# Benjamin-Lee/circkit

Measured on NVIDIA B200. Metric: canonicalize+uniq records/sec, higher is better.
Workload: dtype u8

## Files before the change

### circkit_b200/csrc/ck_kernels.cuh

```cuda
#pragma once
#include "ck_hash.cuh"

namespace ck {

enum : int {
    CLS_W2S = 0,
    CLS_W2M = 1,
    CLS_C2A = 2,
    CLS_C2B = 3,
    CLS_W4 = 4,
    CLS_C4 = 5,
    CLS_W8 = 6,
    CLS_C8 = 7,
    CLS_HUGE = 8,
    CLS_EMPTY = 9,
    CLS_W2L = 10,
    CLS_W2X = 11,
    CLS_COUNT = 12
};
__host__ __device__ constexpr u32 cls_max_n(int c)
{
    return c == CLS_W2S ? 512u : c == CLS_W2M ? 2048u : c == CLS_W2L ? 4096u : c == CLS_W2X ? 8192u : c == CLS_C2A ? 65536u
         : c == CLS_C2B ? 425984u : c == CLS_W4 ? 2048u : c == CLS_C4 ? 212992u : c == CLS_W8 ? 1024u : c == CLS_C8 ? 106496u
         : c == CLS_EMPTY ? 0u : 0xffffffffu;
// ... 316 lines not shown
                    const u32 v = min(16u, rawlen - p);
                    u32 unit = prep_pack16(prep_load16(src16 + (p >> 4), sh, p + 16 < span));
                    if (v < 16) unit &= ~(0xffffffffu >> (2 * v));
                    dst32[p >> 4] = unit;
                }
            }
            continue;
        }
        if (cnt == rawlen && spanA <= 512) {
            const u32 p = 16 * lane;
            if (p < spanA) {
                const u32 lo = p < A ? A - p : 0u, hi = min(16u, spanA - p);
                if (hi - lo == 16) *reinterpret_cast<uint4 *>(gbase + p) = m1;
                else {
                    const u32 valid = (hi >= 16 ? 0xffffu : ((1u << hi) - 1u)) & ~((1u << lo) - 1u);
                    const u32 w[4] = {m1.x, m1.y, m1.z, m1.w};
                    u8 *g = gbase + p;
                    u32 vb = valid;
#pragma unroll
                    for (int i = 0; i < 4; i++)
                        if (((valid >> (4 * i)) & 15u) == 15u) { *reinterpret_cast<u32 *>(g + 4 * i) = w[i]; vb &= ~(15u << (4 * i)); }
                    prep_store_bytes(g, w, vb);
                }
            }
            continue;
        }
        u32 S = pack2 ? 0u : A;
        u32 done = 0;
        for (u32 base = 0; base < rawlen; base += 512) {
            const u32 p = base + 16 * lane;
            uint4 m = make_uint4(0, 0, 0, 0);
            u32 mask = 0;
            if (p < rawlen) {
                u32 f;
                prep_lookup(tab, prep_load16(src16 + (p >> 4), sh, p + 16 < span), 0u, min(16u, rawlen - p), m, f, mask);
            }
            const u32 kc = __popc(mask);
            u32 incl = kc;
#pragma unroll
            for (int d = 1; d < 32; d <<= 1) { const u32 t = __shfl_up_sync(CK_FULL, incl, d); if (lane >= (u32)d) incl += t; }
            const u32 T = __shfl_sync(CK_FULL, incl, 31);
            u32 idx = S + incl - kc;
            __syncwarp();
#pragma unroll
            for (int k = 0; k < 16; k++)
                if ((mask >> k) & 1u) stage[idx++] = (u8)prep_byte(m, k);
            __syncwarp();
            const u32 fill = S + T;
            if (pack2) {
                const u32 U = fill >> 4;
                for (u32 j = lane; j < U; j += 32) dst32[done + j] = prep_pack16(*reinterpret_cast<const uint4 *>(stage + 16 * j));
                const u32 r = fill & 15u;
                u8 c = 0;
                if (lane < r) c = stage[16 * U + lane];
                __syncwarp();
                if (lane < r) stage[lane] = c;
                done += U; S = r;
            } else {
                u8 *g = dstb + done - S;
                for (u32 w = lane; 16 * w < fill; w += 32) {
                    const u32 lo = max(16 * w, S), hi = min(16 * w + 16, fill);
                    if (hi - lo == 16) *reinterpret_cast<uint4 *>(g + 16 * w) = *reinterpret_cast<const uint4 *>(stage + 16 * w);
                    else for (u32 i = lo; i < hi; i++) g[i] = stage[i];
                }
                done += T; S = (u32)((size_t)(dstb + done) & 15u);
            }
        }
        __syncwarp();
        if (pack2 && S && lane == 0)
            dst32[done] = prep_pack16(*reinterpret_cast<const uint4 *>(stage)) & ~(0xffffffffu >> (2 * S));
        __syncwarp();
    }
}

struct ClassifyArgs {
    const u64 *offsets; const u32 *lens; const u8 *lane;
    u32 n_records;
    u32 *keys, *vals;
    u32 *counts;
    u32 direct_mask;
    u32 window_shift;
    u32 top_bit;
};
__global__ void __launch_bounds__(256) k_classify(ClassifyArgs a)
{
    __shared__ u32 cnt[16];
    if (threadIdx.x < 16) cnt[threadIdx.x] = 0;
    __syncthreads();
    const u32 nthreads = gridDim.x * blockDim.x;
    const u32 rounds = (a.n_records + nthreads - 1) / nthreads;
    for (u32 r = 0; r < rounds; r++) {
        const u32 i = r * nthreads + blockIdx.x * blockDim.x + threadIdx.x;
        int cls = -1;
        u32 n = 0;
        if (i < a.n_records) {
            n = a.lens ? a.lens[i] : (u32)(a.offsets[i + 1] - a.offsets[i]);
            const u32 bits = a.lane ? a.lane[i] : 2u;
            if (n == 0) cls = CLS_EMPTY;
            else if (bits == 2) cls = n <= cls_max_n(CLS_W2S) ? CLS_W2S : n <= cls_max_n(CLS_W2M) ? CLS_W2M
                                    : n <= cls_max_n(CLS_W2L) ? CLS_W2L : n <= cls_max_n(CLS_W2X) ? CLS_W2X
                                    : n <= cls_max_n(CLS_C2A) ? CLS_C2A : n <= cls_max_n(CLS_C2B) ? CLS_C2B : CLS_HUGE;
            else if (bits == 4 || bits == 3) cls = n <= cls_max_n(CLS_W4) ? CLS_W4 : n <= cls_max_n(CLS_C4) ? CLS_C4 : CLS_HUGE;
            else cls = n <= cls_max_n(CLS_W8) ? CLS_W8 : n <= cls_max_n(CLS_C8) ? CLS_C8 : CLS_HUGE;
        }
        if (a.direct_mask) {
            const u32 m = __ballot_sync(CK_FULL, cls >= 0 && !((a.direct_mask >> cls) & 1u));
            if (m && lane_id() == (u32)(__ffs(m) - 1)) atomicAdd(cnt + CLS_HUGE, __popc(m));
            continue;
        }
        if (cls >= 0) {
            const u32 msb = 31u - __clz(n | 1u);
            const u32 bin = (msb << 5) | ((((n << (31u - msb)) >> 29) & 3u) << 3);
            u32 key = (cls_rank(cls) << 10) | bin;
            if (a.window_shift < 32u) {
                const bool lane_cls = cls == CLS_W2S || cls == CLS_W2M || cls == CLS_W2L || cls == CLS_W2X;
                const u32 q = (msb << 2) | (((n << (31u - msb)) >> 29) & 3u);
                key = lane_cls ? (((i >> a.window_shift) << 5) | (q > 28u ? q - 28u : 0u)) : (key | (1u << a.top_bit));
            }
            a.keys[i] = key; a.vals[i] = i;
        }
        u32 todo = __ballot_sync(CK_FULL, cls >= 0);
        while (todo) {
            const int c = __shfl_sync(CK_FULL, cls, __ffs(todo) - 1);
            const u32 m = __ballot_sync(CK_FULL, cls == c);
            if (lane_id() == (u32)(__ffs(m) - 1)) atomicAdd(cnt + c, __popc(m));
            todo &= ~m;
        }
    }
    __syncthreads();
    if (threadIdx.x < 16 && cnt[threadIdx.x]) atomicAdd(a.counts + threadIdx.x, cnt[threadIdx.x]);
}
__global__ void k_list_starts(u32 *counts)
{
    if (threadIdx.x == 0) {
        u32 s = 0;
        for (u32 r = 0; r < (u32)CLS_COUNT; r++) {
            const int c = cls_of_rank(r);
            counts[16 + c] = s; counts[48 + c] = s;
            s += counts[c];
        }
        counts[12] = counts[CLS_W2S] + counts[CLS_W2M] + counts[CLS_W2L] + counts[CLS_W2X];
        counts[28] = counts[16 + CLS_W2S];
        counts[13] = counts[CLS_C2A] + counts[CLS_C2B];
        counts[29] = counts[16 + CLS_C2A];
    }
}

__device__ __forceinline__ u32 p2_last_unit(u32 n) { return max((2u * n + 143u) >> 4, (n >> 4) + 5u); }
__device__ __forceinline__ void extend_one(u64 *packed2, const u64 *offsets, const u32 *lens, u32 i, const u64 *dense, u32 dbl, u32 lane)
{
    const u64 off = offsets[i];
    const u32 n = lens ? lens[i] : (u32)(offsets[i + 1] - off);
    if (n == 0) return;
    u32 *U = reinterpret_cast<u32 *>(packed2 + p2_word(off, i, dbl));
    const u32 *S = dense ? reinterpret_cast<const u32 *>(dense + (off >> 5) + i) : U;
    const u32 jn = n >> 4, last = dbl ? p2_last_unit(n) : jn + 4;
    if (n >= 80) {
        for (u32 j = (dense ? 0u : jn) + lane; j <= last; j += 32) {
            const u32 r = (16u * j) % n;
            const u32 q = r >> 4, sh = 2u * (r & 15u);
            u32 w = __funnelshift_l(__ldcg(S + q + 1), __ldcg(S + q), sh);
            if (r + 16u > n) {
                const u32 k = n - r;
                w = (w & ~(0xffffffffu >> (2u * k))) | (__ldcg(S) >> (2u * k));
            }
            U[j] = w;
        }
    } else {
        for (u32 j = (dense ? 0u : jn) + lane; j <= last; j += 32) {
            u32 v = 0;
            for (u32 b = 0; b < 16; b++) {
                const u32 t = (16 * j + b) % n;
                v = (v << 2) | ((__ldcg(S + (t >> 4)) >> (30 - 2 * (t & 15))) & 3u);
            }
            __syncwarp(__activemask());
            U[j] = v;
        }
    }
    __syncwarp();
}
__global__ void __launch_bounds__(256) k_extend_packed2(u64 *packed2, const u64 *offsets, const u32 *lens, const u8 *lane_bits, u32 n_records,
                                                        const u64 *dense, u32 dbl)
{
    const u32 lane = lane_id();
    const u32 gw = (blockIdx.x * blockDim.x + threadIdx.x) >> 5, nw = (gridDim.x * blockDim.x) >> 5;
    if (n_records < 65536u) {
        for (u32 i = gw; i < n_records; i += nw) {
            if (lane_bits && lane_bits[i] != 2) continue;
            extend_one(packed2, offsets, lens, i, dense, dbl, lane);
        }
        return;
    }
    for (u32 i0 = 32u * gw; i0 < n_records; i0 += 32u * nw) {
        const u32 ii = i0 + lane;
        u32 m = __ballot_sync(CK_FULL, ii < n_records && (!lane_bits || lane_bits[ii] == 2));
        while (m) {
            const u32 i = i0 + (u32)__ffs(m) - 1u;
            m &= m - 1u;
            extend_one(packed2, offsets, lens, i, dense, dbl, lane);
        }
    }
}

__global__ void __launch_bounds__(256) k_scatter_lane_bytes(const u8 *lane_bytes, const u64 *lane_offsets, const u64 *offsets, const u32 *lens,
                                                            const u8 *lane_bits, u32 n_records, u8 *bytes)
{
    const u32 lane = lane_id();
    const u32 gw = (blockIdx.x * blockDim.x + threadIdx.x) >> 5, nw = (gridDim.x * blockDim.x) >> 5;
    for (u32 i = gw; i < n_records; i += nw) {
        if (lane_bits[i] == 2) continue;
        const u8 *src = lane_bytes + lane_offsets[i];
        u8 *dst = bytes + offsets[i];
        const u32 n = lens[i];
        for (u32 k = lane; k < n; k += 32) dst[k] = src[k];
    }
}

struct TableArgs {
    TableSlot *slots; u64 nslots;
    u64 *side_first;
    const u64 *hash; const u64 *index;
    u32 stride;
    u64 base_index; u32 n;
    u64 *slot_of;
    u64 *first_out;
    u32 *overflow;
    u64 *keys;
// ... 317 lines not shown
```

### circkit_b200/csrc/ck_lib.cu

```cuda
#include <algorithm>
#include <cstdio>
#include <cstdlib>
#include <cstring>
#include <mutex>
#include <new>
#include <string>
#include <vector>

#include <cub/device/device_radix_sort.cuh>
#include <cub/device/device_scan.cuh>
#include <cub/device/device_select.cuh>
#include <cub/iterator/counting_input_iterator.cuh>

#include "../../include/circkit_b200.h"
#include "ck_kernels.cuh"
#include "ck_warp2.cuh"
#include "ck_lane2.cuh"
#include "ck_stream2.cuh"
#include "ck_stream3.cuh"
#include "ck_seg2.cuh"
#include "ck_lane4.cuh"
#include "ck_synth.cuh"
#include "ck_monomerize.cuh"
#include "ck_fasta.cuh"
// ... 52 lines not shown
struct ExecScratch {
    u32 *tie[CLS_COUNT] = {};
    u64 *seg = nullptr;
    u32 *huge_x = nullptr, *huge_tie = nullptr;
    u64 huge_x_words = 0, huge_tie_words = 0;
    cudaStream_t side_stream[CLS_COUNT] = {};
    cudaEvent_t ev_fork = nullptr, ev_join[CLS_COUNT] = {};
};

struct Slot {
    cudaStream_t stream = nullptr;
    cudaEvent_t inserted = nullptr;
    u8 *d_raw = nullptr; u64 *d_off = nullptr; u64 *d_p2 = nullptr; u8 *d_norm = nullptr; u8 *d_p4 = nullptr;
    u32 *d_len = nullptr; u8 *d_lane = nullptr; u8 *d_out = nullptr; u32 *d_start = nullptr;
    u8 *d_strand = nullptr; u64 *d_hash = nullptr; u64 *d_first = nullptr; u64 *d_slotof = nullptr;
    u32 *d_lists = nullptr; u32 *d_counts = nullptr;
    u64 *d_dense = nullptr; u64 *d_laneoff = nullptr;
    u32 *h_counts = nullptr;
    ExecScratch scr;
    bool busy = false, uniq = false, mono = false;
    bool text = false;
    u32 cmd = 0;
    u8 *d_text = nullptr, *d_frame = nullptr;
    u64 *d_rstart = nullptr, *d_head = nullptr, *d_seq = nullptr, *d_len64 = nullptr, *d_fofs = nullptr, *d_meta = nullptr;
    u32 *d_tiles = nullptr;
    u32 dbl = 1;
    u64 longest = 0;
    u32 *sel = nullptr; u64 *coff = nullptr;
    u32 n = 0, flags = 0; u64 total = 0;
    u64 rec_mark = 0;
    bool defl = false;
    struct Deflate {
        cudaStream_t stream = nullptr;
        u64 cap = 0;
        u8 *buf = nullptr;
        u32 *kA = nullptr, *kB = nullptr, *vA = nullptr, *vB = nullptr;
        u32 *prev8 = nullptr, *prev4 = nullptr;
        u32 *seg = nullptr;
        u32 *out = nullptr, *result = nullptr;
        u32 *h_result = nullptr;
        void *tmp = nullptr; size_t tmp_bytes = 0;
        u64 n = 0;
    } z;
};

struct PeerGroup {
    u32 world = 1, rank = 0, cap = 0;
    u8 *block = nullptr; u64 block_bytes = 0, recv_bytes = 0, ret_bytes = 0;
    void *mapped[32] = {};
    bool exported = false, attached = false;
    u64 epoch[4] = {};
    u32 *pos[2] = {}; u32 *cursors[2] = {}; u64 *slot_of[2] = {};
    u64 *recv(u32 r, u32 slot) const { return reinterpret_cast<u64 *>((u8 *)mapped[r] + CK_PEER_HEADER_BYTES + (u64)slot * recv_bytes); }
    u64 *ret(u32 r, u32 slot) const { return reinterpret_cast<u64 *>((u8 *)mapped[r] + CK_PEER_HEADER_BYTES + 2 * recv_bytes + (u64)slot * ret_bytes); }
    u64 *counts(u32 r, u32 slot) const { return reinterpret_cast<u64 *>(mapped[r]) + CK_PEER_FLAG_WORDS + 32u * slot; }
};

}

struct ck_ctx {
    int device = 0;
    int num_sms = 148;
    ck_config cfg{};
    std::string err;
    Slot slot[2];
    ExecScratch dev_scr;
    cudaEvent_t last_insert = nullptr;
    bool have_last_insert = false;
    TableSlot *table = nullptr; u64 table_slots = 0; u64 *side = nullptr; u32 *d_overflow = nullptr;
    u64 *d_keys = nullptr;
    u64 grow_max = 0, grows = 0;
    u64 known_keys = 0, known_rec = 0, submitted_rec = 0;
    PeerGroup peer;
    std::mutex lib_mu;
    cudaStream_t lib_stream = nullptr;
    u8 *lib_h = nullptr, *lib_d = nullptr; size_t lib_h_bytes = 0, lib_d_bytes = 0;
    ExecScratch lib_scr;
    u64 launches = 0;
    bool attrs_set = false;
    u32 s3_debug = 0;
    bool l4_kernel = true;
    bool seg_kernel = true;
    int lane_kernel = 3;
    bool timing = false;
    std::vector<cudaEvent_t> ev_pairs[CLS_COUNT + 7];
};

namespace {

int fail(ck_ctx *ctx, int code, const char *what, cudaError_t e = cudaSuccess)
{
    std::string m = what;
    if (e != cudaSuccess) { m += ": "; m += cudaGetErrorString(e); }
    if (ctx) ctx->err = m; else g_init_error = m;
    return code;
}
#define CK_CUDA(ctx, call)                                                     \
    do {                                                                       \
        cudaError_t e__ = (call);                                              \
        if (e__ != cudaSuccess) return fail((ctx), CK_ERR_CUDA, #call, e__);   \
    } while (0)

void fill_tables(Tables &t, u8 secret[200])
{
    for (int c = 0; c < 256; c++) t.norm[c] = 'N';
    for (const char *p = "ACGTN-"; *p; p++) t.norm[(u8)*p] = (u8)*p;
    t.norm['a'] = 'A'; t.norm['c'] = 'C'; t.norm['g'] = 'G';
    t.norm['t'] = 'T'; t.norm['u'] = 'T'; t.norm['U'] = 'T';
    t.norm['.'] = '-'; t.norm['~'] = '-';
    t.norm[' '] = 0; t.norm['\t'] = 0; t.norm['\r'] = 0; t.norm['\n'] = 0;
    for (int c = 0; c < 256; c++) t.comp[c] = (u8)c;
    const char *a = "AGCTYRWSKMDVHBN", *b = "TCGARYWSMKHBDVN";
    for (int i = 0; a[i]; i++) { t.comp[(u8)a[i]] = (u8)b[i]; t.comp[(u8)a[i] + 32] = (u8)(b[i] + 32); }
    const char *alpha = "-ABCDGHKMNRSTVWY";
    for (int c = 0; c < 256; c++) t.code4[c] = 0xff;
    for (int i = 0; i < 16; i++) { t.sym4[i] = (u8)alpha[i]; t.code4[(u8)alpha[i]] = (u8)i; }
    for (int i = 0; i < 16; i++) t.comp4[i] = t.code4[t.comp[t.sym4[i]]];
    static const u8 sec[192] = {
        0xb8, 0xfe, 0x6c, 0x39, 0x23, 0xa4, 0x4b, 0xbe, 0x7c, 0x01, 0x81, 0x2c, 0xf7, 0x21, 0xad, 0x1c,
        0xde, 0xd4, 0x6d, 0xe9, 0x83, 0x90, 0x97, 0xdb, 0x72, 0x40, 0xa4, 0xa4, 0xb7, 0xb3, 0x67, 0x1f,
        0xcb, 0x79, 0xe6, 0x4e, 0xcc, 0xc0, 0xe5, 0x78, 0x82, 0x5a, 0xd0, 0x7d, 0xcc, 0xff, 0x72, 0x21,
        0xb8, 0x08, 0x46, 0x74, 0xf7, 0x43, 0x24, 0x8e, 0xe0, 0x35, 0x90, 0xe6, 0x81, 0x3a, 0x26, 0x4c,
        0x3c, 0x28, 0x52, 0xbb, 0x91, 0xc3, 0x00, 0xcb, 0x88, 0xd0, 0x65, 0x8b, 0x1b, 0x53, 0x2e, 0xa3,
        0x71, 0x64, 0x48, 0x97, 0xa2, 0x0d, 0xf9, 0x4e, 0x38, 0x19, 0xef, 0x46, 0xa9, 0xde, 0xac, 0xd8,
        0xa8, 0xfa, 0x76, 0x3f, 0xe3, 0x9c, 0x34, 0x3f, 0xf9, 0xdc, 0xbb, 0xc7, 0xc7, 0x0b, 0x4f, 0x1d,
        0x8a, 0x51, 0xe0, 0x4b, 0xcd, 0xb4, 0x59, 0x31, 0xc8, 0x9f, 0x7e, 0xc9, 0xd9, 0x78, 0x73, 0x64,
        0xea, 0xc5, 0xac, 0x83, 0x34, 0xd3, 0xeb, 0xc3, 0xc5, 0x81, 0xa0, 0xff, 0xfa, 0x13, 0x63, 0xeb,
        0x17, 0x0d, 0xdd, 0x51, 0xb7, 0xf0, 0xda, 0x49, 0xd3, 0x16, 0x55, 0x26, 0x29, 0xd4, 0x68, 0x9e,
        0x2b, 0x16, 0xbe, 0x58, 0x7d, 0x47, 0xa1, 0xfc, 0x8f, 0xf8, 0xb8, 0xd1, 0x7a, 0xd0, 0x31, 0xce,
        0x45, 0xcb, 0x3a, 0x8f, 0x95, 0x16, 0x04, 0x28, 0xaf, 0xd7, 0xfb, 0xca, 0xbb, 0x4b, 0x40, 0x7e,
    };
    memset(secret, 0, 200);
    memcpy(secret, sec, 192);
}

int alloc_scratch(ck_ctx *ctx, ExecScratch &s)
{
    CK_CUDA(ctx, cudaEventCreateWithFlags(&s.ev_fork, cudaEventDisableTiming));
    for (int c = 0; c < CLS_COUNT; c++) {
        CK_CUDA(ctx, cudaStreamCreateWithFlags(&s.side_stream[c], cudaStreamNonBlocking));
        CK_CUDA(ctx, cudaEventCreateWithFlags(&s.ev_join[c], cudaEventDisableTiming));
    }
    CK_CUDA(ctx, cudaMalloc(&s.seg, (size_t)2 * ctx->num_sms * CK_SEG_WARPS * CK_SEG_SCRATCH_U64 * 8));
    for (int c = 0; c < CLS_COUNT; c++) {
        if (kCls[c].bits == 0) continue;
        const u64 groups = (u64)kCls[c].ctas_per_sm * ctx->num_sms * (kCls[c].cta ? 1u : kCls[c].threads / 32u);
        CK_CUDA(ctx, cudaMalloc(&s.tie[c], groups * cls_tie_words(c) * 4));
    }
    return CK_OK;
}
void free_scratch(ExecScratch &s)
{
    for (int c = 0; c < CLS_COUNT; c++) {
        if (s.tie[c]) cudaFree(s.tie[c]);
        if (s.side_stream[c]) cudaStreamDestroy(s.side_stream[c]);
        if (s.ev_join[c]) cudaEventDestroy(s.ev_join[c]);
        s.tie[c] = nullptr; s.side_stream[c] = nullptr; s.ev_join[c] = nullptr;
    }
    if (s.ev_fork) cudaEventDestroy(s.ev_fork);
    if (s.seg) cudaFree(s.seg);
    if (s.huge_x) cudaFree(s.huge_x);
    if (s.huge_tie) cudaFree(s.huge_tie);
    s.huge_x = s.huge_tie = nullptr; s.huge_x_words = s.huge_tie_words = 0;
    s.ev_fork = nullptr; s.seg = nullptr;
}

template <typename K> int set_smem(ck_ctx *ctx, K kernel, u32 bytes)
{
    if (bytes > 48 * 1024) CK_CUDA(ctx, cudaFuncSetAttribute(kernel, cudaFuncAttributeMaxDynamicSharedMemorySize, (int)bytes));
    return CK_OK;
}
void s2_launch(ck_ctx *ctx, cudaStream_t st, const CanonArgs &a, int v)
{
    if (ctx->lane_kernel != 2 && a.p2_dbl) {
        const u32 g3 = 2u * (u32)ctx->num_sms, th3 = 32u * CK_S3_WARPS, sm3 = CK_S3_WARPS * CK_S3_WARP_BYTES;
#define CK_S3(V) k_canon_s3<V><<<g3, th3, sm3, st>>>(a)
        switch (v) {
        case 0: CK_S3(0); break; case 1: CK_S3(1); break; case 2: CK_S3(2); break; case 3: CK_S3(3); break;
        case 4: CK_S3(4); break; case 5: CK_S3(5); break; case 6: CK_S3(6); break; default: CK_S3(7);
        }
#undef CK_S3
        return;
    }
    const u32 g = 2u * (u32)ctx->num_sms, th = 32u * CK_S2_WARPS, sm = CK_S2_WARPS * CK_S2_WARP_BYTES;
#define CK_S2(V) k_canon_s2<V><<<g, th, sm, st>>>(a)
    switch (v) {
    case 0: CK_S2(0); break; case 1: CK_S2(1); break; case 2: CK_S2(2); break; case 3: CK_S2(3); break;
    case 4: CK_S2(4); break; case 5: CK_S2(5); break; case 6: CK_S2(6); break; default: CK_S2(7);
    }
#undef CK_S2
}

int set_attrs(ck_ctx *ctx)
{
    if (ctx->attrs_set) return CK_OK;
    int rc;
    if ((rc = set_smem(ctx, k_canon_cta<2, false>, cls_smem_bytes(CLS_C2B)))) return rc;
    if ((rc = set_smem(ctx, k_canon_cta<4, false>, cls_smem_bytes(CLS_C4)))) return rc;
    if ((rc = set_smem(ctx, k_canon_cta<8, false>, cls_smem_bytes(CLS_C8)))) return rc;
    const u32 s2 = CK_S2_WARPS * CK_S2_WARP_BYTES;
    if ((rc = set_smem(ctx, k_canon_s2<0>, s2)) || (rc = set_smem(ctx, k_canon_s2<1>, s2)) || (rc = set_smem(ctx, k_canon_s2<2>, s2)) ||
        (rc = set_smem(ctx, k_canon_s2<3>, s2)) || (rc = set_smem(ctx, k_canon_s2<4>, s2)) || (rc = set_smem(ctx, k_canon_s2<5>, s2)) ||
        (rc = set_smem(ctx, k_canon_s2<6>, s2)) || (rc = set_smem(ctx, k_canon_s2<7>, s2))) return rc;
    const u32 s3 = CK_S3_WARPS * CK_S3_WARP_BYTES;
    if ((rc = set_smem(ctx, k_canon_s3<0>, s3)) || (rc = set_smem(ctx, k_canon_s3<1>, s3)) || (rc = set_smem(ctx, k_canon_s3<2>, s3)) ||
        (rc = set_smem(ctx, k_canon_s3<3>, s3)) || (rc = set_smem(ctx, k_canon_s3<4>, s3)) || (rc = set_smem(ctx, k_canon_s3<5>, s3)) ||
        (rc = set_smem(ctx, k_canon_s3<6>, s3)) || (rc = set_smem(ctx, k_canon_s3<7>, s3))) return rc;
    const u32 l4 = CK_L4_WARPS * CK_L4_WARP_BYTES;
    if ((rc = set_smem(ctx, k_canon_l4<0>, l4)) || (rc = set_smem(ctx, k_canon_l4<1>, l4)) || (rc = set_smem(ctx, k_canon_l4<2>, l4)) ||
        (rc = set_smem(ctx, k_canon_l4<3>, l4))) return rc;
    ctx->attrs_set = true;
    return CK_OK;
}

struct CanonIO {
    const u64 *packed2; const u8 *bytes; const u64 *offsets; const u32 *lens; const u8 *lane;
    u32 n; u32 mode;
    u32 dbl = 1;
    u64 longest = 0;
    u8 *p4 = nullptr;
    u8 *out; u32 *out_start; u8 *out_strand; u64 *out_hash;
    u32 *lists; u64 lists_bytes;
    u32 *counts;
};

u64 lists_bytes_for(u64 n) { return ((16 * (n + 4) + 24 * (n + 4) + 255) & ~255ull) + (1ull << 20); }

int run_canon(ck_ctx *ctx, cudaStream_t st, ExecScratch &scr, const CanonIO &io, u32 class_mask)
{
    if (io.n == 0) return CK_OK;
    int rc = set_attrs(ctx);
    if (rc) return rc;
    CK_CUDA(ctx, cudaMemsetAsync(io.counts, 0, 64 * sizeof(u32), st));
    int only = -1;
    if (class_mask && (class_mask & (class_mask - 1)) == 0)
        for (int c = 0; c < CLS_COUNT; c++) if (class_mask == (1u << c)) only = c;
    const u64 stride = ((u64)io.n + 4) & ~3ull;
    u32 *k0 = io.lists, *k1 = k0 + stride, *v0 = k1 + stride, *v1 = v0 + stride;
    if (io.lists_bytes < 16 * stride) return fail(ctx, CK_ERR_ARG, "sort workspace too small");
    const bool fastv = io.packed2 && !(io.mode & 1u) && (!io.out || (io.mode & 2u)) && io.out_start && io.out_strand;
    u32 window_shift = 32, top_bit = 13;
    if (fastv && only < 0) {
        window_shift = 16;
        u32 wbits = 0;
        while ((((u64)io.n - 1) >> window_shift) >> wbits) wbits++;
        top_bit = std::max(14u, 5u + wbits);
    }
    const bool l4_run = fastv && only < 0 && ctx->l4_kernel && io.p4 && io.lane && io.bytes && (!class_mask || (class_mask & (1u << CLS_W4)));
    if (l4_run) {
        cudaEvent_t e0 = nullptr, e1 = nullptr;
        if (ctx->timing) { CK_CUDA(ctx, cudaEventCreate(&e0)); CK_CUDA(ctx, cudaEventCreate(&e1)); CK_CUDA(ctx, cudaEventRecord(e0, st)); }
        k_pack4<<<std::min<u32>((io.n + 15) / 16, 16u * (u32)ctx->num_sms), 256, 0, st>>>(io.bytes, io.offsets, io.lens, const_cast<u8 *>(io.lane), io.n, io.p4);
        if (ctx->timing) { CK_CUDA(ctx, cudaEventRecord(e1, st)); ctx->ev_pairs[CLS_COUNT + 5].push_back(e0); ctx->ev_pairs[CLS_COUNT + 5].push_back(e1); }
        ctx->launches++;
    }
    const int sort_bits = (int)top_bit + 1;
    const bool lane_checks = fastv && only >= 0 && io.lane == nullptr &&
                             (only == CLS_W2S || only == CLS_W2M || only == CLS_W2L || only == CLS_W2X);
    if (!lane_checks) {
        ClassifyArgs ca{io.offsets, io.lens, io.lane, io.n, k0, v0, io.counts, only >= 0 ? (1u << only) : 0u, window_shift, top_bit};
        k_classify<<<std::min<u32>((io.n + 255) / 256, 16u * (u32)ctx->num_sms), 256, 0, st>>>(ca);
        ctx->launches++;
    }
    const u32 *sorted = nullptr;
    u32 *retry = v0;
    if (only < 0) {
        cub::DoubleBuffer<u32> keys(k0, k1), vals(v0, v1);
        void *tmp = v1 + stride;
        size_t tmp_bytes = (size_t)(io.lists_bytes - 16 * stride), need = 0;
        cub::DeviceRadixSort::SortPairs(nullptr, need, keys, vals, (int)io.n, 0, sort_bits, st);
        if (need > tmp_bytes) return fail(ctx, CK_ERR_ARG, "sort workspace too small");
        CK_CUDA(ctx, cub::DeviceRadixSort::SortPairs(tmp, need, keys, vals, (int)io.n, 0, sort_bits, st));
        sorted = vals.Current();
        retry = vals.Alternate();
        k_list_starts<<<1, 32, 0, st>>>(io.counts);
        ctx->launches += 2;
    }
    const u32 lane_classes = (1u << CLS_W2S) | (1u << CLS_W2M) | (1u << CLS_W2L) | (1u << CLS_W2X);
    auto timed = [&](int slot, cudaEvent_t &e0, cudaEvent_t &e1, bool begin, cudaStream_t on) -> cudaError_t {
        if (!ctx->timing) return cudaSuccess;
        if (begin) {
            cudaError_t e = cudaEventCreate(&e0); if (e != cudaSuccess) return e;
            e = cudaEventCreate(&e1); if (e != cudaSuccess) return e;
            return cudaEventRecord(e0, on);
        }
        ctx->ev_pairs[slot].push_back(e0); ctx->ev_pairs[slot].push_back(e1);
        return cudaEventRecord(e1, on);
    };
    auto base_args = [&](int c) {
        CanonArgs a{};
        a.packed2 = io.packed2; a.p2_dbl = io.dbl; a.bytes = io.bytes; a.offsets = io.offsets; a.lens = io.lens;
        a.max_n = cls_max_n(c); a.min_n = cls_min_n(c);
        a.out = io.out; a.out_start = io.out_start; a.out_strand = io.out_strand; a.out_hash = io.out_hash;
        a.scratch = scr.tie[c]; a.scratch_stride = kCls[c].bits ? cls_tie_words(c) : 0;
        a.smem_units = kCls[c].bits ? cls_units(c) : 0; a.xglobal = nullptr; a.mode = io.mode;
        a.retry = retry; a.retry_counts = io.counts + 32;
        return a;
    };
    const bool lane_run = fastv && (only >= 0 ? ((lane_classes >> only) & 1u) != 0 : (!class_mask || (class_mask & lane_classes)));
    if (lane_run) {
        CanonArgs a = base_args(only >= 0 ? only : CLS_W2S);
        if (only >= 0) { a.list = nullptr; a.count = nullptr; a.n_direct = io.n; }
        else { a.list = sorted; a.count = io.counts + 12; a.n_direct = 0; a.min_n = 1; a.max_n = cls_max_n(CLS_W2X); }
        const int v = (a.out_hash ? CK_W2_HASH : 0) | (a.out ? CK_W2_OUT : 0) | (a.list ? CK_W2_LIST : 0);
        a.mode |= ctx->s3_debug;
        cudaEvent_t e0 = nullptr, e1 = nullptr;
        CK_CUDA(ctx, timed(CLS_COUNT, e0, e1, true, st));
        s2_launch(ctx, st, a, v);
        CK_CUDA(ctx, timed(CLS_COUNT, e0, e1, false, st));
        ctx->launches++;
    }
    const u32 seg_classes = (1u << CLS_C2A) | (1u << CLS_C2B);
    const bool seg_run = fastv && only < 0 && ctx->seg_kernel && io.dbl && (!class_mask || (class_mask & seg_classes));
    if (seg_run) {
        CanonArgs a = base_args(CLS_C2A);
        a.list = sorted; a.count = io.counts + 13; a.n_direct = 0;
        const u32 g = 2u * (u32)ctx->num_sms, th = 32u * CK_SEG_WARPS, sm = CK_SEG_WARPS * CK_SEG_WARP_BYTES;
        cudaEvent_t e0 = nullptr, e1 = nullptr;
        CK_CUDA(ctx, timed(CLS_COUNT + 3, e0, e1, true, st));
        switch ((a.out_hash ? CK_W2_HASH : 0) | (a.out ? CK_W2_OUT : 0)) {
        case 0: k_canon_seg<0><<<g, th, sm, st>>>(a, scr.seg); break;
        case 1: k_canon_seg<1><<<g, th, sm, st>>>(a, scr.seg); break;
        case 2: k_canon_seg<2><<<g, th, sm, st>>>(a, scr.seg); break;
        default: k_canon_seg<3><<<g, th, sm, st>>>(a, scr.seg); break;
        }
        CK_CUDA(ctx, timed(CLS_COUNT + 3, e0, e1, false, st));
        ctx->launches++;
    }
    if (l4_run) {
        CanonArgs a = base_args(CLS_W4);
        a.list = sorted; a.count = io.counts + CLS_W4; a.n_direct = 0;
        const u32 g = 2u * (u32)ctx->num_sms, th = 32u * CK_L4_WARPS, sm = CK_L4_WARPS * CK_L4_WARP_BYTES;
        cudaEvent_t e0 = nullptr, e1 = nullptr;
        CK_CUDA(ctx, timed(CLS_COUNT + 4, e0, e1, true, st));
        switch ((a.out_hash ? CK_W2_HASH : 0) | (a.out ? CK_W2_OUT : 0)) {
        case 0: k_canon_l4<0><<<g, th, sm, st>>>(a, io.p4, io.lane); break;
        case 1: k_canon_l4<1><<<g, th, sm, st>>>(a, io.p4, io.lane); break;
        case 2: k_canon_l4<2><<<g, th, sm, st>>>(a, io.p4, io.lane); break;
        default: k_canon_l4<3><<<g, th, sm, st>>>(a, io.p4, io.lane); break;
        }
        CK_CUDA(ctx, timed(CLS_COUNT + 4, e0, e1, false, st));
        ctx->launches++;
    }
    u32 to_launch = 0;
    for (int c = 0; c < CLS_COUNT; c++)
        if (c != CLS_HUGE && !(class_mask && !(class_mask & (1u << c)))) to_launch++;
    const bool fork = scr.ev_fork != nullptr && to_launch >= 2;
    if (fork) CK_CUDA(ctx, cudaEventRecord(scr.ev_fork, st));
    u32 joined = 0;
    for (int c = 0; c < CLS_COUNT; c++) {
        if (c == CLS_HUGE) continue;
        if (class_mask && !(class_mask & (1u << c))) continue;
        CanonArgs a = base_args(c);
        const bool is_lane_cls = ((lane_classes >> c) & 1u) != 0;
        if ((lane_run && is_lane_cls) || (seg_run && ((seg_classes >> c) & 1u)) || (l4_run && c == CLS_W4)) { a.list = retry; a.count = io.counts + 32 + c; a.n_direct = 0; }
        else if (only >= 0) { a.list = nullptr; a.count = nullptr; a.n_direct = io.n; }
        else { a.list = sorted; a.count = io.counts + c; a.n_direct = 0; }
        const u32 grid = kCls[c].ctas_per_sm * (u32)ctx->num_sms, thr = kCls[c].threads;
        const u32 smem = kCls[c].bits ? cls_smem_bytes(c) : 0;
        cudaEvent_t e0 = nullptr, e1 = nullptr;
        const bool side = fork && (!kCls[c].cta || (seg_run && ((seg_classes >> c) & 1u)));
// ... 384 lines not shown
{
    if (!ctx) return CK_ERR_ARG;
    if (!b) return fail(ctx, CK_ERR_ARG, "null batch");
    const u32 n_records = b->n_records;
    int rc = submit_check(ctx, slot, b->offsets, n_records, flags | CK_F_PACKED_IN, uniq, true);
    if (rc) return rc;
    Slot &s = ctx->slot[slot];
    if (n_records == 0) return submit_empty(ctx, s, base_index);
    if (!b->packed2 || !b->lens || !b->lane) return fail(ctx, CK_ERR_ARG, "null batch pointers");
    if (b->lane_bytes_total && (!b->lane_bytes || !b->lane_offsets)) return fail(ctx, CK_ERR_ARG, "byte-lane records without lane_bytes / lane_offsets");
    if (b->lane_bytes_total > ctx->cfg.max_batch_bytes) return fail(ctx, CK_ERR_ARG, "lane_bytes exceed max_batch_bytes");
    cudaStream_t st = s.stream;
    CK_CUDA(ctx, cudaSetDevice(ctx->device));
    if (uniq && !ctx->peer.attached && (rc = table_reserve(ctx, s, n_records))) return rc;
    CK_CUDA(ctx, cudaMemcpyAsync(s.d_off, b->offsets, (size_t)(n_records + 1) * 8, cudaMemcpyHostToDevice, st));
    CK_CUDA(ctx, cudaMemcpyAsync(s.d_len, b->lens, (size_t)n_records * 4, cudaMemcpyHostToDevice, st));
    CK_CUDA(ctx, cudaMemcpyAsync(s.d_lane, b->lane, (size_t)n_records, cudaMemcpyHostToDevice, st));
    CK_CUDA(ctx, cudaMemcpyAsync(s.d_dense, b->packed2, (size_t)ck_pack2_words(s.total, n_records) * 8, cudaMemcpyHostToDevice, st));
    k_extend_packed2<<<extend_grid(ctx, n_records), 256, 0, st>>>(s.d_p2, s.d_off, s.d_len, s.d_lane, n_records, s.d_dense, s.dbl);
    ctx->launches++;
    if (b->lane_bytes_total) {
        CK_CUDA(ctx, cudaMemcpyAsync(s.d_laneoff, b->lane_offsets, (size_t)(n_records + 1) * 8, cudaMemcpyHostToDevice, st));
        CK_CUDA(ctx, cudaMemcpyAsync(s.d_raw, b->lane_bytes, (size_t)b->lane_bytes_total, cudaMemcpyHostToDevice, st));
        k_scatter_lane_bytes<<<extend_grid(ctx, n_records), 256, 0, st>>>(s.d_raw, s.d_laneoff, s.d_off, s.d_len, s.d_lane, n_records, s.d_norm);
        ctx->launches++;
    }
    return submit_tail(ctx, s, true, base_index);
}

int wait_common(ck_ctx *ctx, int slot, bool uniq, uint8_t *out_bytes, uint32_t *out_len, uint32_t *out_start,
                uint8_t *out_strand, uint64_t *out_hash, uint64_t *out_first)
{
    if (!ctx) return CK_ERR_ARG;
    if (slot < 0 || slot > 1) return fail(ctx, CK_ERR_ARG, "slot must be 0 or 1");
    Slot &s = ctx->slot[slot];
    if (!s.busy || s.uniq != uniq || s.mono || s.text || s.defl) return fail(ctx, CK_ERR_STATE, "no matching submit on this slot");
    s.busy = false;
    if (s.n == 0) {
        if (uniq && ctx->peer.attached && ctx->peer.world > 1) CK_CUDA(ctx, cudaStreamSynchronize(s.stream));
        return CK_OK;
    }
    cudaStream_t st = s.stream;
    const size_t n = s.n;
    if (out_bytes && !(s.flags & CK_F_NO_BYTES) && s.total)
        CK_CUDA(ctx, cudaMemcpyAsync(out_bytes, s.d_out, (s.flags & CK_F_ALIGNED_OUT) ? ck_out_arena_bytes(s.total, s.n) : s.total,
                                     cudaMemcpyDeviceToHost, st));
    if (out_len) CK_CUDA(ctx, cudaMemcpyAsync(out_len, s.d_len, n * 4, cudaMemcpyDeviceToHost, st));
    if (out_start) CK_CUDA(ctx, cudaMemcpyAsync(out_start, s.d_start, n * 4, cudaMemcpyDeviceToHost, st));
    if (out_strand) CK_CUDA(ctx, cudaMemcpyAsync(out_strand, s.d_strand, n, cudaMemcpyDeviceToHost, st));
    if (out_hash) CK_CUDA(ctx, cudaMemcpyAsync(out_hash, s.d_hash, n * 8, cudaMemcpyDeviceToHost, st));
    if (out_first && uniq) CK_CUDA(ctx, cudaMemcpyAsync(out_first, s.d_first, n * 8, cudaMemcpyDeviceToHost, st));
    CK_CUDA(ctx, cudaStreamSynchronize(st));
    if (uniq) note_keys(ctx, s);
    if (s.h_counts[CLS_HUGE]) return fail(ctx, CK_ERR_TOO_LONG, "batch holds a record beyond the staged-length classes");
    if (uniq && s.h_counts[16]) return fail(ctx, CK_ERR_TABLE_FULL, "uniq table is full; raise table_capacity");
    return CK_OK;
}

}

static bool table_view(void *table, u64 bytes, TableSlot *&slots, u64 &nslots, u64 *&side, u32 *&overflow)
{
    if (!table || bytes < 64 + sizeof(TableSlot) * 16) return false;
    nslots = (bytes - 64) / sizeof(TableSlot);
    side = (u64 *)table; overflow = (u32 *)((u8 *)table + 8);
    slots = (TableSlot *)((u8 *)table + 64);
    return true;
}

extern "C" {

int ck_init(const ck_config *cfg, ck_ctx **out)
{
    if (!cfg || !out) return fail(nullptr, CK_ERR_ARG, "null argument");
    *out = nullptr;
    ck_ctx *ctx = new (std::nothrow) ck_ctx();
    if (!ctx) return fail(nullptr, CK_ERR_ARG, "out of host memory");
    ctx->cfg = *cfg;
    ctx->device = cfg->device;
    if (const char *dbg = getenv("CK_S3_DEBUG")) ctx->s3_debug = (u32)strtoul(dbg, nullptr, 0) & 0xff00u;
    if (const char *sk = getenv("CK_SEG_KERNEL")) ctx->seg_kernel = atoi(sk) != 0;
    if (const char *lk = getenv("CK_L4_KERNEL")) ctx->l4_kernel = atoi(lk) != 0;
    if (const char *lk = getenv("CK_LANE_KERNEL")) ctx->lane_kernel = atoi(lk) == 2 ? 2 : 3;
#define CK_INIT(call)                                                                          \
    do {                                                                                       \
        cudaError_t e__ = (call);                                                              \
        if (e__ != cudaSuccess) { fail(nullptr, CK_ERR_CUDA, #call, e__); ck_destroy(ctx); return CK_ERR_CUDA; } \
    } while (0)
    CK_INIT(cudaSetDevice(ctx->device));
    cudaDeviceProp prop;
    CK_INIT(cudaGetDeviceProperties(&prop, ctx->device));
    ctx->num_sms = prop.multiProcessorCount;
    Tables t; u8 secret[200];
    fill_tables(t, secret);
    CK_INIT(cudaMemcpyToSymbol(c_tab, &t, sizeof(t)));
    CK_INIT(cudaMemcpyToSymbol(c_secret, secret, sizeof(secret)));
    {
        u64 last[8], merge[8], mid[16];
        for (int i = 0; i < 8; i++) { memcpy(&last[i], secret + 121 + 8 * i, 8); memcpy(&merge[i], secret + 11 + 8 * i, 8); }
        for (int i = 0; i < 14; i++) memcpy(&mid[i], secret + 3 + 8 * i, 8);
        memcpy(&mid[14], secret + 119, 8); memcpy(&mid[15], secret + 127, 8);
        CK_INIT(cudaMemcpyToSymbol(c_lastsec, last, sizeof(last)));
        CK_INIT(cudaMemcpyToSymbol(c_mergesec, merge, sizeof(merge)));
        CK_INIT(cudaMemcpyToSymbol(c_midsec, mid, sizeof(mid)));
    }
    if (alloc_scratch(ctx, ctx->dev_scr)) { g_init_error = ctx->err; ck_destroy(ctx); return CK_ERR_CUDA; }
    if (alloc_scratch(ctx, ctx->lib_scr)) { g_init_error = ctx->err; ck_destroy(ctx); return CK_ERR_CUDA; }
    CK_INIT(cudaStreamCreateWithFlags(&ctx->lib_stream, cudaStreamNonBlocking));
    const u64 B = cfg->max_batch_bytes, R = cfg->max_batch_records;
    if (B || R) {
        for (int k = 0; k < 2; k++) {
            Slot &s = ctx->slot[k];
            CK_INIT(cudaStreamCreateWithFlags(&s.stream, cudaStreamNonBlocking));
            CK_INIT(cudaEventCreateWithFlags(&s.inserted, cudaEventDisableTiming));
            CK_INIT(cudaMalloc(&s.d_raw, B + 16));
            CK_INIT(cudaMalloc(&s.d_norm, B + 16));
            CK_INIT(cudaMalloc(&s.d_out, out_bytes_total(B, R) + 64));
            CK_INIT(cudaMalloc(&s.d_p2, p2_words(B, R) * 8));
            CK_INIT(cudaMalloc(&s.d_p4, p4_bytes_total(B, R)));
            CK_INIT(cudaMalloc(&s.d_off, (R + 1) * 8));
            CK_INIT(cudaMalloc(&s.d_len, (R + 1) * 4));
            CK_INIT(cudaMalloc(&s.d_lane, R + 1));
            CK_INIT(cudaMalloc(&s.d_start, (R + 1) * 4));
            CK_INIT(cudaMalloc(&s.d_strand, R + 1));
            CK_INIT(cudaMalloc(&s.d_hash, (R + 1) * 8));
            CK_INIT(cudaMalloc(&s.d_first, (R + 1) * 8));
            CK_INIT(cudaMalloc(&s.d_slotof, (R + 1) * 8));
            CK_INIT(cudaMalloc(&s.d_lists, lists_bytes_for(R)));
            CK_INIT(cudaMalloc(&s.d_counts, 64 * 4));
            CK_INIT(cudaMalloc(&s.d_dense, ((B >> 5) + R + 2) * 8));
            CK_INIT(cudaMalloc(&s.d_laneoff, (R + 1) * 8));
            CK_INIT(cudaMallocHost(&s.h_counts, 32 * 4));
            memset(s.h_counts, 0, 32 * 4);
            if (alloc_scratch(ctx, s.scr)) { g_init_error = ctx->err; ck_destroy(ctx); return CK_ERR_CUDA; }
        }
    }
    CK_INIT(cudaMalloc(&ctx->side, 8));
    CK_INIT(cudaMalloc(&ctx->d_overflow, 16));
    CK_INIT(cudaMemset(ctx->d_overflow, 0, 16));
    ctx->d_keys = reinterpret_cast<u64 *>(ctx->d_overflow + 2);
    if (cfg->table_capacity) {
        ctx->table_slots = table_slots_for(cfg->table_capacity);
        CK_INIT(cudaMalloc(&ctx->table, ctx->table_slots * sizeof(TableSlot)));
        k_table_clear<<<ctx->num_sms * 4, 256>>>(ctx->table, ctx->table_slots, ctx->side);
        CK_INIT(cudaGetLastError());
    }
    CK_INIT(cudaDeviceSynchronize());
#undef CK_INIT
    *out = ctx;
    return CK_OK;
}

void ck_destroy(ck_ctx *ctx)
{
    if (!ctx) return;
    cudaSetDevice(ctx->device);
    cudaDeviceSynchronize();
    for (int k = 0; k < 2; k++) {
        Slot &s = ctx->slot[k];
        void *ptrs[] = {s.d_raw, s.d_off, s.d_p2, s.d_norm, s.d_len, s.d_lane, s.d_out, s.d_start, s.d_strand,
                        s.d_hash, s.d_first, s.d_slotof, s.d_lists, s.d_counts, s.d_dense, s.d_laneoff, s.d_p4,
                        s.d_text, s.d_frame, s.d_rstart, s.d_head, s.d_seq, s.d_len64, s.d_fofs, s.d_meta, s.d_tiles};
        for (void *p : ptrs) if (p) cudaFree(p);
        if (s.h_counts) cudaFreeHost(s.h_counts);
        if (s.stream) cudaStreamDestroy(s.stream);
        {
// ... 940 lines not shown
```

Baseline: 1.456 billion.

## Replace classify+radix sort with per-window counting-sort list builder for lane classes

When all requested classes are contiguous 2-bit lane classes, a single kernel now builds the per-window length-binned record list, replacing the classify kernel, CUB radix sort and list-starts launch. Each block counts length bins for one window in shared memory, reserves output space with an atomic, and scatters record indices. This removes global key/value writes and a multi-pass sort, but ordering across windows now depends on atomic order and requires large dynamic shared memory per block.

```diff
diff --git a/circkit_b200/csrc/ck_kernels.cuh b/circkit_b200/csrc/ck_kernels.cuh
--- a/circkit_b200/csrc/ck_kernels.cuh
+++ b/circkit_b200/csrc/ck_kernels.cuh
@@ -422,6 +422,12 @@
     u32 window_shift;
     u32 top_bit;
 };
+__device__ __forceinline__ u32 len_bin(u32 n)
+{
+    const u32 msb = 31u - __clz(n | 1u);
+    const u32 q = (msb << 2) | (((n << (31u - msb)) >> 29) & 3u);
+    return q > 28u ? q - 28u : 0u;
+}
 __global__ void __launch_bounds__(256) k_classify(ClassifyArgs a)
 {
     __shared__ u32 cnt[16];
@@ -454,8 +460,7 @@
             u32 key = (cls_rank(cls) << 10) | bin;
             if (a.window_shift < 32u) {
                 const bool lane_cls = cls == CLS_W2S || cls == CLS_W2M || cls == CLS_W2L || cls == CLS_W2X;
-                const u32 q = (msb << 2) | (((n << (31u - msb)) >> 29) & 3u);
-                key = lane_cls ? (((i >> a.window_shift) << 5) | (q > 28u ? q - 28u : 0u)) : (key | (1u << a.top_bit));
+                key = lane_cls ? (((i >> a.window_shift) << 5) | len_bin(n)) : (key | (1u << a.top_bit));
             }
             a.keys[i] = key; a.vals[i] = i;
         }
@@ -483,6 +488,46 @@
         counts[28] = counts[16 + CLS_W2S];
         counts[13] = counts[CLS_C2A] + counts[CLS_C2B];
         counts[29] = counts[16 + CLS_C2A];
+    }
+}
+
+__global__ void __launch_bounds__(1024) k_window_list(const u64 *offsets, const u32 *lens, u32 n_records, u32 window_shift,
+                                                      u32 min_n, u32 max_n, u32 *list, u32 *counts, u32 retry_stride)
+{
+    extern __shared__ u8 wbin[];
+    __shared__ u32 hist[32];
+    const u32 w0 = blockIdx.x << window_shift, len = min(n_records - w0, 1u << window_shift);
+    if (threadIdx.x < 32) hist[threadIdx.x] = 0;
+    if (blockIdx.x == 0 && threadIdx.x < 4) counts[48 + cls_of_rank(threadIdx.x)] = threadIdx.x * retry_stride;
+    __syncthreads();
+    u32 outside = 0;
+#pragma unroll 8
+    for (u32 i = threadIdx.x; i < len; i += blockDim.x) {
+        const u32 r = w0 + i;
+        const u32 n = lens ? lens[r] : (u32)(offsets[r + 1] - offsets[r]);
+        const bool in = n >= min_n && n <= max_n;
+        const u32 b = len_bin(n);
+        wbin[i] = in ? (u8)b : (u8)0xff;
+        outside += in ? 0u : 1u;
+        if (in) atomicAdd(hist + b, 1u);
+    }
+    outside = __reduce_add_sync(CK_FULL, outside);
+    if (outside && lane_id() == 0) atomicAdd(counts + CLS_HUGE, outside);
+    __syncthreads();
+    if (threadIdx.x < 32) {
+        const u32 c = hist[threadIdx.x];
+        u32 inc = c;
+#pragma unroll
+        for (u32 d = 1; d < 32; d <<= 1) { const u32 y = __shfl_up_sync(CK_FULL, inc, d); if (threadIdx.x >= d) inc += y; }
+        u32 b0 = 0;
+        if (threadIdx.x == 31) b0 = atomicAdd(counts + 12, inc);
+        b0 = __shfl_sync(CK_FULL, b0, 31);
+        hist[threadIdx.x] = b0 + inc - c;
+    }
+    __syncthreads();
+    for (u32 i = threadIdx.x; i < len; i += blockDim.x) {
+        const u32 b = wbin[i];
+        if (b != 0xffu) list[atomicAdd(hist + b, 1u)] = w0 + i;
     }
 }
 
diff --git a/circkit_b200/csrc/ck_lib.cu b/circkit_b200/csrc/ck_lib.cu
--- a/circkit_b200/csrc/ck_lib.cu
+++ b/circkit_b200/csrc/ck_lib.cu
@@ -158,6 +158,7 @@
     bool l4_kernel = true;
     bool seg_kernel = true;
     int lane_kernel = 3;
+    bool window_list = true;
     bool timing = false;
     std::vector<cudaEvent_t> ev_pairs[CLS_COUNT + 7];
 };
@@ -282,6 +283,7 @@
     if ((rc = set_smem(ctx, k_canon_s3<0>, s3)) || (rc = set_smem(ctx, k_canon_s3<1>, s3)) || (rc = set_smem(ctx, k_canon_s3<2>, s3)) ||
         (rc = set_smem(ctx, k_canon_s3<3>, s3)) || (rc = set_smem(ctx, k_canon_s3<4>, s3)) || (rc = set_smem(ctx, k_canon_s3<5>, s3)) ||
         (rc = set_smem(ctx, k_canon_s3<6>, s3)) || (rc = set_smem(ctx, k_canon_s3<7>, s3))) return rc;
+    if ((rc = set_smem(ctx, k_window_list, 1u << 16))) return rc;
     const u32 l4 = CK_L4_WARPS * CK_L4_WARP_BYTES;
     if ((rc = set_smem(ctx, k_canon_l4<0>, l4)) || (rc = set_smem(ctx, k_canon_l4<1>, l4)) || (rc = set_smem(ctx, k_canon_l4<2>, l4)) ||
         (rc = set_smem(ctx, k_canon_l4<3>, l4))) return rc;
@@ -331,16 +333,30 @@
         ctx->launches++;
     }
     const int sort_bits = (int)top_bit + 1;
+    const u32 lane_classes = (1u << CLS_W2S) | (1u << CLS_W2M) | (1u << CLS_W2L) | (1u << CLS_W2X);
     const bool lane_checks = fastv && only >= 0 && io.lane == nullptr &&
                              (only == CLS_W2S || only == CLS_W2M || only == CLS_W2L || only == CLS_W2X);
-    if (!lane_checks) {
+    u32 rank_lo = CLS_COUNT, rank_hi = 0;
+    for (int c = 0; c < CLS_COUNT; c++)
+        if ((class_mask >> c) & 1u) { rank_lo = std::min(rank_lo, cls_rank(c)); rank_hi = std::max(rank_hi, cls_rank(c)); }
+    const bool window_list = fastv && only < 0 && io.lane == nullptr && ctx->window_list && class_mask && !(class_mask & ~lane_classes) &&
+                             (u32)__builtin_popcount(class_mask) == rank_hi - rank_lo + 1 && stride < (1u << 30) &&
+                             io.lists_bytes >= 20 * stride;
+    if (!lane_checks && !window_list) {
         ClassifyArgs ca{io.offsets, io.lens, io.lane, io.n, k0, v0, io.counts, only >= 0 ? (1u << only) : 0u, window_shift, top_bit};
         k_classify<<<std::min<u32>((io.n + 255) / 256, 16u * (u32)ctx->num_sms), 256, 0, st>>>(ca);
         ctx->launches++;
     }
     const u32 *sorted = nullptr;
     u32 *retry = v0;
-    if (only < 0) {
+    if (window_list) {
+        const u32 windows = (u32)(((u64)io.n + (1u << window_shift) - 1) >> window_shift);
+        k_window_list<<<windows, 1024, 1u << window_shift, st>>>(io.offsets, io.lens, io.n, window_shift, cls_min_n(cls_of_rank(rank_lo)),
+                                                                  cls_max_n(cls_of_rank(rank_hi)), k0, io.counts, (u32)stride);
+        sorted = k0;
+        retry = k1;
+        ctx->launches++;
+    } else if (only < 0) {
         cub::DoubleBuffer<u32> keys(k0, k1), vals(v0, v1);
         void *tmp = v1 + stride;
         size_t tmp_bytes = (size_t)(io.lists_bytes - 16 * stride), need = 0;
@@ -352,7 +368,6 @@
         k_list_starts<<<1, 32, 0, st>>>(io.counts);
         ctx->launches += 2;
     }
-    const u32 lane_classes = (1u << CLS_W2S) | (1u << CLS_W2M) | (1u << CLS_W2L) | (1u << CLS_W2X);
     auto timed = [&](int slot, cudaEvent_t &e0, cudaEvent_t &e1, bool begin, cudaStream_t on) -> cudaError_t {
         if (!ctx->timing) return cudaSuccess;
         if (begin) {
@@ -903,6 +918,7 @@
     if (const char *sk = getenv("CK_SEG_KERNEL")) ctx->seg_kernel = atoi(sk) != 0;
     if (const char *lk = getenv("CK_L4_KERNEL")) ctx->l4_kernel = atoi(lk) != 0;
     if (const char *lk = getenv("CK_LANE_KERNEL")) ctx->lane_kernel = atoi(lk) == 2 ? 2 : 3;
+    if (const char *wl = getenv("CK_WINDOW_LIST")) ctx->window_list = atoi(wl) != 0;
 #define CK_INIT(call)                                                                          \
     do {                                                                                       \
         cudaError_t e__ = (call);                                                              \
```

Measured after the change: 1.500 billion, median of 6. +3.0%, better.
